# raphaelsulzer/PixelsPointsPolygons

Hardware: NVIDIA B200
Metric: pillar_encode_tiles_per_sec (higher is better)
Workload: dtype f16 operands, f32 accumulate, f32 in/out

## Files before the change

### pixelspointspolygons_b200/csrc/voxelize.cu

```cuda
#include <type_traits>

#include "p3p_internal.cuh"

namespace p3p {

#ifdef P3P_TIMELINE
__device__ unsigned long long g_timeline[8192][16];
__device__ __forceinline__ void tl_stamp(int cta, int slot) {
    if (threadIdx.x == 0 && cta < 8192) {
        unsigned long long t;
        asm volatile("mov.u64 %0, %%globaltimer;" : "=l"(t));
        g_timeline[cta][slot] = t;
    }
}
#define TL(cta, slot) tl_stamp(cta, slot)
extern "C" int p3p_debug_timeline(unsigned long long* host, int ctas) {
    return (int)cudaMemcpyFromSymbol(host, g_timeline, sizeof(unsigned long long) * 16 * (size_t)ctas);
}
#else
#define TL(cta, slot)
#endif

namespace {

constexpr int kThreads = kVoxThreads;
constexpr int kWarps = kThreads / 32;
constexpr int kIters = kMaxChunkPoints / kThreads;

struct ChunkLoc {
    int b;
    int c;
    int nchunks;
    int gstart;
    long long p0;
    long long lo, hi;
    unsigned sat;
};

__device__ __forceinline__ unsigned atoms_add_u16(uint32_t addr, int pred) {
    unsigned r;
    const unsigned sh = (addr & 2u) * 8u;
    asm volatile(
        "{\n .reg .pred p;\n setp.ne.b32 p, %3, 0;\n mov.b32 %0, 0;\n @p atom.shared.add.u32 %0, [%1], %2;\n}"
        : "=r"(r)
        : "r"(addr & ~3u), "r"(1u << sh), "r"(pred)
        : "memory");
    return (r >> sh) & 0xFFFFu;
}

__device__ __forceinline__ unsigned ld_acquire(const unsigned* p) {
    unsigned v;
    asm volatile("ld.acquire.gpu.global.u32 %0, [%1];" : "=r"(v) : "l"(p) : "memory");
    return v;
}
__device__ __forceinline__ void st_release(unsigned* p, unsigned v) {
    asm volatile("st.release.gpu.global.u32 [%0], %1;" ::"l"(p), "r"(v) : "memory");
}

__device__ void locate_chunk(int g, const int64_t* __restrict__ offsets, int B, int S, int phase, ChunkLoc* out) {
    const int lane = threadIdx.x & 31;
    if (B <= 32) {
        long long o0 = 0, o1 = 0;
        if (lane < B) { o0 = offsets[lane]; o1 = offsets[lane + 1]; }
        const long long a0 = o0 - ((o0 - phase) & 3ll);
        const long long n = o1 > o0 ? o1 - a0 : 0;
        const int nc = (int)((n + S - 1) / S);
        int incl = nc;
#pragma unroll
        for (int o = 1; o < 32; o <<= 1) {
            const int v = __shfl_up_sync(0xffffffffu, incl, o);
            if (lane >= o) incl += v;
        }
        const int total = __shfl_sync(0xffffffffu, incl, 31);
        if (g >= total) {
            if (lane == 0) out->b = -1;
            return;
        }
        int lo = 0, hi = __reduce_max_sync(0xffffffffu, nc) - 1;
        while (lo < hi) {
            const int mid = (lo + hi + 1) >> 1;
            if (__reduce_add_sync(0xffffffffu, nc < mid ? nc : mid) <= g) lo = mid; else hi = mid - 1;
        }
        const int c = lo;
        const int r = g - __reduce_add_sync(0xffffffffu, nc < c ? nc : c);
        const bool has = nc > c;
        const unsigned bal = __ballot_sync(0xffffffffu, has);
        if (has && __popc(bal & ((1u << lane) - 1u)) == r) {
            out->b = lane;
            out->c = c;
            out->nchunks = nc;
            out->gstart = incl - nc;
            out->p0 = a0 + (long long)c * S;
            out->lo = o0;
            out->hi = o1;
        }
        return;
    }
    int base = 0;
    bool found = false;
    for (int t0 = 0; t0 < B && !found; t0 += 32) {
        const int t = t0 + lane;
        long long o0 = 0, o1 = 0;
        if (t < B) { o0 = offsets[t]; o1 = offsets[t + 1]; }
        const long long a0 = o0 - ((o0 - phase) & 3ll);
        const long long n = o1 > o0 ? o1 - a0 : 0;
        const int nc = (int)((n + S - 1) / S);
        int incl = nc;
#pragma unroll
        for (int o = 1; o < 32; o <<= 1) {
            const int v = __shfl_up_sync(0xffffffffu, incl, o);
            if (lane >= o) incl += v;
        }
        const int excl = base + incl - nc;
        const bool mine = (t < B) && (g >= excl) && (g < excl + nc);
        const unsigned bal = __ballot_sync(0xffffffffu, mine);
        if (bal) {
            found = true;
            if (mine) {
                out->b = t;
                out->c = g - excl;
                out->nchunks = nc;
                out->gstart = excl;
                out->p0 = a0 + (long long)(g - excl) * S;
                out->lo = o0;
                out->hi = o1;
            }
        }
        base += __shfl_sync(0xffffffffu, incl, 31);
    }
    if (!found && lane == 0) out->b = -1;
}

__device__ __forceinline__ int block_exclusive_scan(int v, int* warp_tot, int* total) {
    const int lane = threadIdx.x & 31, w = threadIdx.x >> 5;
    int incl = v;
#pragma unroll
    for (int o = 1; o < 32; o <<= 1) {
        const int t = __shfl_up_sync(0xffffffffu, incl, o);
        if (lane >= o) incl += t;
    }
    __syncthreads();
    if (lane == 31) warp_tot[w] = incl;
    __syncthreads();
    int off = 0, tot = 0;
#pragma unroll
    for (int i = 0; i < kWarps; ++i) {
        const int t = warp_tot[i];
        if (i < w) off += t;
        tot += t;
    }
    *total = tot;
    return off + incl - v;
}

__device__ void write_empty_tile(const GridDev& g, const WsPtrs& ws, int b) {
    const int HW = g.ny * g.nx;
    for (int i = threadIdx.x; i < HW; i += kThreads) {
        ws.owner[(size_t)b * HW + i] = -1;
        ws.cell_desc[(size_t)b * HW + i] = -1;
    }
    if (threadIdx.x == 0) ws.num_pil[b] = 0;
}

__device__ void plan_tile(const GridDev& g, const WsPtrs& ws, int b, int Keff, int* scratch, int* warp_tot) {
    const int K = g.num_keys, HW = g.ny * g.nx, M = g.M, tid = threadIdx.x;
    int* n_s = scratch;
    int* cell_s = n_s + K;
    int* rkey_s = cell_s + K;
    int* rn_s = rkey_s + K;
    int* owner_s = rn_s + K;
    const int* totals = ws.totals + (size_t)b * K;
    const float4* slots = ws.slots + (size_t)b * K * M;
    const uint8_t* edge = ws.edge + (size_t)b * K;
    for (int k0 = 0; k0 < Keff; k0 += kThreads * 8) {
        int t[8];
        uint8_t e[8];
#pragma unroll
        for (int u = 0; u < 8; ++u) {
            const int k = k0 + u * kThreads + tid;
            t[u] = 0; e[u] = 0;
            if (k < Keff) { t[u] = __ldcg(totals + k); e[u] = __ldcg(edge + k); }
        }
#pragma unroll
        for (int u = 0; u < 8; ++u) {
            const int k = k0 + u * kThreads + tid;
            if (k >= Keff) continue;
            int cell = -1;
            const int n = t[u] < M ? t[u] : M;
            if (n > 0) {
                int cx, cy, cz;
                if (e[u]) {
                    float4 best = __ldcg(slots + (size_t)k * M);
                    for (int i = 1; i < n; ++i) {
                        const float4 p = __ldcg(slots + (size_t)k * M + i);
                        if (__float_as_int(p.w) < __float_as_int(best.w)) best = p;
                    }
                    point_cell(g, best.x, best.y, best.z, cx, cy, cz);
                } else {
                    cz = k / g.stride2;
                    const int rem = k - cz * g.stride2;
                    cy = rem / g.stride1;
                    cx = rem - cy * g.stride1;
                }
                if (cy < g.nv[1] && cx < g.nv[0]) cell = cx | (cy << 10) | (cz << 20);
            }
            n_s[k] = n;
            cell_s[k] = cell;
        }
    }
    for (int i = tid; i < HW; i += kThreads) owner_s[i] = -1;
    __syncthreads();
    const int per = (Keff + kThreads - 1) / kThreads;
    const int k0 = tid * per, k1 = (k0 + per < Keff) ? k0 + per : Keff;
    int cnt = 0;
    for (int k = k0; k < k1; ++k) cnt += (n_s[k] > 0);
    int total_runs;
    int ord = block_exclusive_scan(cnt, warp_tot, &total_runs);
    int cnt2 = 0;
    for (int k = k0; k < k1; ++k) {
        if (n_s[k] > 0) {
            const int r = ord++;
            if (r >= g.Vmax) cell_s[k] = -1;
        }
        cnt2 += (cell_s[k] >= 0);
    }
    int total_pil;
    int ord2 = block_exclusive_scan(cnt2, warp_tot, &total_pil);
    for (int k = k0; k < k1; ++k) {
        const int st = cell_s[k];
        if (st < 0) continue;
        const int r = ord2++;
        const size_t pi = (size_t)b * g.Vmax + r;
        const int n = n_s[k];
        ws.pil_key[pi] = k;
        ws.pil_n[pi] = n;
        ws.pil_coord[pi] = st;
        rkey_s[r] = k;
        rn_s[r] = n;
        const int cx = st & 1023, cy = (st >> 10) & 1023;
        atomicMax(&owner_s[cy * g.nx + cx], r);
    }
    if (tid == 0) ws.num_pil[b] = total_pil;
    __syncthreads();
    for (int i = tid; i < HW; i += kThreads) {
        const int o = owner_s[i];
        ws.owner[(size_t)b * HW + i] = o;
        ws.cell_desc[(size_t)b * HW + i] = (o >= 0) ? (rkey_s[o] | (rn_s[o] << 16)) : -1;
    }
}

constexpr int kKeyBits = 13;
constexpr unsigned kKeyMask = (1u << kKeyBits) - 1u;
static_assert(kMaxKeys <= (1 << kKeyBits), "key field too narrow");
static_assert(kMaxChunkPoints * 8 < 65536, "8 chunk rows must add up inside 16-bit lanes");
constexpr int kGroups = kIters / 4;
#ifndef P3P_CROSS_BATCH
#define P3P_CROSS_BATCH 256
#endif
constexpr int kCrossBatch = P3P_CROSS_BATCH;
constexpr int kCells = kGroups * kWarps;
static_assert(kMaxChunkPoints / kCells <= 255, "points of a cell must fit the 8-bit fields of the boundary word");
constexpr unsigned kCrossFlag = 0x8000u;

template <bool kFast>
__global__ void __launch_bounds__(kThreads, kVoxCtasPerSm)
voxelize_kernel(const float* __restrict__ pts, int stride_arg, const int64_t* __restrict__ offsets, int B, GridDev g, int S, WsPtrs ws, int32_t* __restrict__ point_hash, int need_plan, int pdl_from) {
    extern __shared__ __align__(16) unsigned char smem_raw[];
    const int K = g.num_keys;
    const int Kp = ws.key_stride;
    uint16_t* ctot_s = reinterpret_cast<uint16_t*>(smem_raw);
    uint16_t* base_s = ctot_s + Kp;
    uint16_t* need_s = base_s + Kp;
    unsigned* bnd_s = reinterpret_cast<unsigned*>(need_s + Kp);
    uint16_t* cell_s = reinterpret_cast<uint16_t*>(bnd_s + kCrossBatch);
    __shared__ ChunkLoc loc;
    __shared__ int s_ticket, s_last, s_runs[2], s_ncross;
    __shared__ int warp_tot[kWarps];

    const int tid = threadIdx.x, lane = tid & 31;
    const int stride = kFast ? 3 : stride_arg;
    TL(blockIdx.x, 0);
    if (tid == 0) { s_ticket = (int)atomicAdd(ws.sync, 1u); s_ncross = 0; }
    {
        uint4* h4 = reinterpret_cast<uint4*>(ctot_s);
        for (int i = tid; i < Kp / 8; i += kThreads) h4[i] = make_uint4(0, 0, 0, 0);
    }
    __syncthreads();
    const int ticket = s_ticket;
    if (ticket >= pdl_from) asm volatile("griddepcontrol.launch_dependents;" ::: "memory");
    unsigned* flags = ws.sync + 1;
    unsigned* tile_done = flags + ws.max_chunks;
    unsigned* tile_sat = tile_done + B;
    if (tid < 32) {
        locate_chunk(ticket, offsets, B, S, kFast ? (int)((reinterpret_cast<uintptr_t>(pts) >> 2) & 3u) : 0, &loc);
        __syncwarp();
        if (lane == 0 && loc.b >= 0) loc.sat = __ldcg(tile_sat + loc.b);
    }
    if (ticket < B && offsets[ticket + 1] <= offsets[ticket]) write_empty_tile(g, ws, ticket);
    __syncthreads();
    if (loc.b < 0) return;
    TL(blockIdx.x, 1);

    uint8_t* edge = ws.edge + (size_t)loc.b * K;
    const int M = g.M;
    const unsigned sat_word = loc.sat;
    const bool saturated = sat_word != 0u && (int)(0x7fffffffu - sat_word) < loc.c;

    int pk[kIters];
    int hi_key = 0;
    const long long lo = loc.lo, hi = loc.hi;
    const uint32_t ctot_sa = smem_u32(ctot_s);
    const bool interior = kFast && S == kMaxChunkPoints && loc.p0 >= lo && loc.p0 + S <= hi;
    auto load_group = [&](int gi, float (&x)[4], float (&y)[4], float (&z)[4]) {
        const long long p = loc.p0 + 4ll * (kThreads * gi + tid);
        if (kFast && p >= lo && p + 4 <= hi) {
            const float4* q = reinterpret_cast<const float4*>(pts + p * 3);
            const float4 a = __ldg(q), b = __ldg(q + 1), c = __ldg(q + 2);
            x[0] = a.x; y[0] = a.y; z[0] = a.z; x[1] = a.w; y[1] = b.x; z[1] = b.y;
            x[2] = b.z; y[2] = b.w; z[2] = c.x; x[3] = c.y; y[3] = c.z; z[3] = c.w;
        } else {
#pragma unroll
            for (int e = 0; e < 4; ++e) {
                x[e] = y[e] = z[e] = __int_as_float(0x7fc00000);
                if (p + e >= lo && p + e < hi) {
                    const float* q = pts + (p + e) * stride;
                    x[e] = __ldg(q); y[e] = __ldg(q + 1); z[e] = __ldg(q + 2);
                }
            }
        }
    };
    {
        unsigned edge_bits = 0;
        int kmax = -1;
        auto hash_group = [&](int gi, const float (&x)[4], const float (&y)[4], const float (&z)[4]) {
#pragma unroll
            for (int e = 0; e < 4; ++e) {
                bool on_edge;
                int k = point_key<!kFast>(g, x[e], y[e], z[e], on_edge);
                if (!kFast && point_hash) {
                    const long long p = loc.p0 + 4ll * (kThreads * gi + tid) + e;
                    if (p >= lo && p < hi) point_hash[p] = k;
                }
                edge_bits |= on_edge ? (1u << (4 * gi + e)) : 0u;
                kmax = k > kmax ? k : kmax;
                if (saturated && k < g.num_cells) k = -1;
                pk[4 * gi + e] = k;
            }
        };
        if (interior) {
            const float4* q = reinterpret_cast<const float4*>(pts + (loc.p0 + 4ll * tid) * 3);
            float4 v[kGroups][3];
#pragma unroll
            for (int gi = 0; gi < kGroups; ++gi) {
#pragma unroll
                for (int u = 0; u < 3; ++u) v[gi][u] = __ldg(q + (size_t)gi * (kThreads * 3) + u);
            }
#pragma unroll
            for (int gi = 0; gi < kGroups; ++gi) {
                const float4 a = v[gi][0], b = v[gi][1], c = v[gi][2];
                const float x[4] = {a.x, a.w, b.z, c.y}, y[4] = {a.y, b.x, b.w, c.z}, z[4] = {a.z, b.y, c.x, c.w};
                hash_group(gi, x, y, z);
            }
        } else {
#pragma unroll
            for (int gi = 0; gi < kGroups; ++gi) {
                if (4 * kThreads * gi < S) {
                    float x[4], y[4], z[4];
                    load_group(gi, x, y, z);
                    hash_group(gi, x, y, z);
                } else {
#pragma unroll
                    for (int e = 0; e < 4; ++e) pk[4 * gi + e] = -1;
                }
            }
        }
        hi_key |= ((kmax >= g.num_cells) ? 1 : 0) | (edge_bits ? 3 : 0);
        if (edge_bits) {
#pragma unroll
            for (int j = 0; j < kIters; ++j)
                if (((edge_bits >> j) & 1u) && pk[j] >= 0) edge[pk[j]] = 1;
        }
        TL(blockIdx.x, 2);
#pragma unroll
        for (int j = 0; j < kIters; ++j) {
            const int k = pk[j];
            const int act = k >= 0 ? 1 : 0;
            const unsigned old = atoms_add_u16(ctot_sa + 2u * (unsigned)(act ? k : 0), act);
            if (act) pk[j] = k | (int)(old << kKeyBits);
        }
    }
    hi_key = (__syncthreads_or(hi_key & 1) ? 1 : 0) | (__syncthreads_or(hi_key & 2) ? 2 : 0);
    TL(blockIdx.x, 3);
    if (tid < 2) s_runs[tid] = 0;
    const int Kreg = (g.num_cells + 7) / 8 * 8 < Kp ? (g.num_cells + 7) / 8 * 8 : Kp;
    {
        uint4* dst = reinterpret_cast<uint4*>(ws.chunk_hist + (size_t)(loc.gstart + loc.c) * Kp);
        for (int k8 = tid; k8 < Kp / 8; k8 += kThreads) dst[k8] = reinterpret_cast<const uint4*>(ctot_s)[k8];
        __syncthreads();
        if (tid == 0) {
            __threadfence();
            st_release(flags + loc.gstart + loc.c, 1u | ((unsigned)hi_key << 1));
        }
        TL(blockIdx.x, 4);
        int hi_before = 0;
        for (int cc = tid; cc < loc.c; cc += kThreads) {
            unsigned f;
            while ((f = ld_acquire(flags + loc.gstart + cc)) == 0u) {
            }
            hi_before |= (int)(f >> 1);
        }
        hi_key |= (__syncthreads_or(hi_before & 1) ? 1 : 0) | (__syncthreads_or(hi_before & 2) ? 2 : 0);
    }
    TL(blockIdx.x, 5);
    const bool last_chunk = (loc.c == loc.nchunks - 1);
    const int Kuse = (hi_key & 1) ? Kp : Kreg;
    int open_keys = 0;
    int all_full = 1;
    for (int k8 = tid; k8 < Kp / 8; k8 += kThreads) {
        unsigned acc[8] = {0, 0, 0, 0, 0, 0, 0, 0};
        if (k8 * 8 < Kuse && !(saturated && k8 * 8 + 8 <= g.num_cells)) {
            const uint4* src = reinterpret_cast<const uint4*>(ws.chunk_hist + (size_t)loc.gstart * Kp) + k8;
            const size_t row = (size_t)Kp / 8;
            const uint4* rp = src;
            auto add_rows = [&](const uint4 (&v)[8]) {
                uint4 sum = v[0];
#pragma unroll
                for (int u = 1; u < 8; ++u) { sum.x += v[u].x; sum.y += v[u].y; sum.z += v[u].z; sum.w += v[u].w; }
                acc[0] += sum.x & 0xFFFFu; acc[1] += sum.x >> 16; acc[2] += sum.y & 0xFFFFu; acc[3] += sum.y >> 16;
                acc[4] += sum.z & 0xFFFFu; acc[5] += sum.z >> 16; acc[6] += sum.w & 0xFFFFu; acc[7] += sum.w >> 16;
            };
            int c0 = 0;
            for (; c0 + 8 <= loc.c; c0 += 8, rp += 8 * row) {
                uint4 v[8];
#pragma unroll
                for (int u = 0; u < 8; ++u) v[u] = __ldcg(rp + u * row);
                add_rows(v);
            }
            if (c0 < loc.c) {
                uint4 v[8];
#pragma unroll
                for (int u = 0; u < 8; ++u) v[u] = (c0 + u < loc.c) ? __ldcg(rp + u * row) : make_uint4(0, 0, 0, 0);
                add_rows(v);
            }
        }
#pragma unroll
        for (int u = 0; u < 8; ++u) {
            const int k = k8 * 8 + u;
            const unsigned own = ctot_s[k];
            unsigned pre = acc[u];
            if (saturated && k < g.num_cells) pre = (unsigned)M;
            unsigned st = pre < (unsigned)M ? pre : (unsigned)M;
            if (own > 0 && pre < (unsigned)M) {
                open_keys = 1;
                if (pre + own > (unsigned)M) {
                    const unsigned id = (unsigned)atomicAdd(&s_ncross, 1);
                    need_s[id] = (uint16_t)((unsigned)M - pre);
                    st = kCrossFlag | id;
                }
            }
            base_s[k] = (uint16_t)st;
            if (k < g.num_cells && pre + own < (unsigned)M) all_full = 0;
            if (last_chunk) {
                const unsigned tot = pre + own;
                if (k < K) ws.totals[(size_t)loc.b * K + k] = (int)tot;
                ctot_s[k] = (uint16_t)(tot < (unsigned)M ? tot : (unsigned)M);
            }
        }
    }
    open_keys = __syncthreads_or(open_keys);
    all_full = __syncthreads_and(all_full);
    if (all_full && !saturated && !last_chunk && tid == 0) atomicMax(tile_sat + loc.b, 0x7fffffffu - (unsigned)loc.c);
    TL(blockIdx.x, 6);
    if (last_chunk) {
        int direct = 0, hi_ok = 0;
        if (!need_plan && !(hi_key & 2)) {
            int r = 0, h = 0;
            for (int k = tid; k < Kuse && k < K; k += kThreads) {
                const int nz = ctot_s[k] > 0 ? 1 : 0;
                if (k < g.num_cells) r += nz; else h += nz;
            }
            r = __reduce_add_sync(0xffffffffu, r);
            h = __reduce_add_sync(0xffffffffu, h);
            if (lane == 0) { atomicAdd(&s_runs[0], r); atomicAdd(&s_runs[1], h); }
            __syncthreads();
            const int R = s_runs[0], H = s_runs[1];
            hi_ok = (R + H <= g.Vmax) ? 1 : 0;
            direct = (R <= g.Vmax) && (H == 0 || hi_ok || R == g.Vmax);
        }
        if (direct) {
            const int HW = g.ny * g.nx;
            const int top = hi_ok ? g.ext[2] : g.ext[2] - 1;
            for (int cell = tid; cell < HW; cell += kThreads) {
                const int cy = cell / g.nx, cx = cell - cy * g.nx;
                int d = -1;
                if (cx < g.nv[0] && cy < g.nv[1]) {
                    for (int cz = top; cz >= 0; --cz) {
                        const int k = cx + cy * g.stride1 + cz * g.stride2;
                        const int n = (k < Kuse && k < K) ? (int)ctot_s[k] : 0;
                        if (n > 0) { d = k | (n << 16); break; }
                    }
                }
                ws.cell_desc[(size_t)loc.b * HW + cell] = d;
            }
        }
        if (tid == 0) ws.tile_hi[loc.b] = (hi_key & 1) | (direct << 1);
    }
    float4* tile_slots = ws.slots + (size_t)loc.b * K * M;
    unsigned xmask = 0;
    const int w = tid >> 5;
    if (open_keys) {
#pragma unroll
        for (int j = 0; j < kIters; ++j) {
            if (pk[j] >= 0) {
                const unsigned key = (unsigned)pk[j] & kKeyMask;
                const unsigned st = base_s[key];
                if (st & kCrossFlag) xmask |= 1u << j;
                else if (st < (unsigned)M) pk[j] = (int)(key | ((st + ((unsigned)pk[j] >> kKeyBits)) << kKeyBits));
                else pk[j] = -1;
            }
        }
    } else {
#pragma unroll
        for (int j = 0; j < kIters; ++j) pk[j] = -1;
    }
    TL(blockIdx.x, 7);
    const int ncross = s_ncross;
    for (int c0 = 0; c0 < ncross; c0 += kCrossBatch) {
        const int nb = ncross - c0 < kCrossBatch ? ncross - c0 : kCrossBatch;
        {
            uint4* c4 = reinterpret_cast<uint4*>(cell_s);
            for (int i = tid; i < kCells * kCrossBatch / 8; i += kThreads) c4[i] = make_uint4(0, 0, 0, 0);
        }
        __syncthreads();
        const uint32_t cell_sa = smem_u32(cell_s);
        unsigned bmask = 0;
        if (xmask) {
#pragma unroll
            for (int j = 0; j < kIters; ++j) {
                if ((xmask >> j) & 1u) {
                    const unsigned key = (unsigned)pk[j] & kKeyMask;
                    const int id = (int)(base_s[key] & (kCrossFlag - 1u)) - c0;
                    if (id >= 0 && id < nb) {
                        bmask |= 1u << j;
                        const unsigned cell = (unsigned)((j >> 2) * kWarps + w);
                        const unsigned local = atoms_add_u16(cell_sa + 2u * (cell * kCrossBatch + (unsigned)id), 1);
                        pk[j] = (int)(key | (local << kKeyBits));
                    }
                }
            }
        }
        __syncthreads();
        for (int id = tid; id < nb; id += kThreads) {
            const unsigned need = need_s[c0 + id];
            unsigned P = 0, bnd = 0;
            bool found = false;
#pragma unroll 8
            for (int c = 0; c < kCells; ++c) {
                const unsigned v = cell_s[c * kCrossBatch + id];
                cell_s[c * kCrossBatch + id] = (uint16_t)P;
                if (!found && P + v >= need) { found = true; bnd = (unsigned)c | ((need - P) << 8) | (v << 16); }
                P += v;
            }
            bnd_s[id] = bnd;
        }
        __syncthreads();
        if (__any_sync(0xffffffffu, bmask != 0)) {
#pragma unroll
            for (int gi = 0; gi < kGroups; ++gi) {
                const unsigned cell = (unsigned)(gi * kWarps + w);
                unsigned flag = 0;
                int keyv[4];
#pragma unroll
                for (int e = 0; e < 4; ++e) {
                    const int j = 4 * gi + e;
                    keyv[e] = -1;
                    if ((bmask >> j) & 1u) {
                        const unsigned key = (unsigned)pk[j] & kKeyMask, local = (unsigned)pk[j] >> kKeyBits;
                        const int id = (int)(base_s[key] & (kCrossFlag - 1u)) - c0;
                        const unsigned bnd = bnd_s[id], bc = bnd & 0xFFu, rem = (bnd >> 8) & 0xFFu, cnt = bnd >> 16;
                        const unsigned pre = (unsigned)M - need_s[c0 + id];
                        const unsigned P = cell_s[cell * kCrossBatch + (unsigned)id];
                        if (cell < bc || (cell == bc && rem == cnt)) pk[j] = (int)(key | ((pre + P + local) << kKeyBits));
                        else if (cell > bc) pk[j] = -1;
                        else { flag |= 1u << e; keyv[e] = (int)key; }
                    }
                }
                unsigned pending = __ballot_sync(0xffffffffu, flag != 0);
                while (pending) {
                    const int leader = __ffs(pending) - 1;
                    const int mine = (flag & 1u) ? keyv[0] : ((flag & 2u) ? keyv[1] : ((flag & 4u) ? keyv[2] : keyv[3]));
                    const int kk = __shfl_sync(0xffffffffu, mine, leader);
                    unsigned b[4], m = 0;
#pragma unroll
                    for (int e = 0; e < 4; ++e) {
                        const bool hit = ((flag >> e) & 1u) && keyv[e] == kk;
                        m |= hit ? (1u << e) : 0u;
                        b[e] = __ballot_sync(0xffffffffu, hit);
                    }
                    if (m) {
                        const int id = (int)(base_s[kk] & (kCrossFlag - 1u)) - c0;
                        const unsigned rem = (bnd_s[id] >> 8) & 0xFFu;
                        const unsigned pre = (unsigned)M - need_s[c0 + id];
                        const unsigned P = cell_s[cell * kCrossBatch + (unsigned)id];
                        const unsigned lt = (1u << lane) - 1u;
                        unsigned below = (unsigned)(__popc(b[0] & lt) + __popc(b[1] & lt) + __popc(b[2] & lt) + __popc(b[3] & lt));
#pragma unroll
                        for (int e = 0; e < 4; ++e) {
                            if ((m >> e) & 1u) {
                                pk[4 * gi + e] = below < rem ? (int)((unsigned)kk | ((pre + P + below) << kKeyBits)) : -1;
                                ++below;
                            }
                        }
                        flag &= ~m;
                    }
                    pending = __ballot_sync(0xffffffffu, flag != 0);
                }
            }
        }
        xmask &= ~bmask;
        __syncthreads();
    }
    TL(blockIdx.x, 8);
    {
        unsigned live = 0;
#pragma unroll
        for (int j = 0; j < kIters; ++j) live |= (pk[j] >= 0) ? (1u << (j >> 2)) : 0u;
        if (interior) {
            const float4* q = reinterpret_cast<const float4*>(pts + (loc.p0 + 4ll * tid) * 3);
#pragma unroll
            for (int h = 0; h < kGroups; h += 2) {
                float4 v[2][3];
#pragma unroll
                for (int g2 = 0; g2 < 2; ++g2) {
                    if (h + g2 < kGroups && ((live >> (h + g2)) & 1u)) {
#pragma unroll
                        for (int u = 0; u < 3; ++u) v[g2][u] = __ldg(q + (size_t)(h + g2) * (kThreads * 3) + u);
                    }
                }
#pragma unroll
                for (int g2 = 0; g2 < 2; ++g2) {
                    const int gi = (h + g2 < kGroups) ? h + g2 : kGroups - 1;
                    if (h + g2 < kGroups && ((live >> gi) & 1u)) {
                        const float4 a = v[g2][0], b = v[g2][1], c = v[g2][2];
                        const float x[4] = {a.x, a.w, b.z, c.y}, y[4] = {a.y, b.x, b.w, c.z}, z[4] = {a.z, b.y, c.x, c.w};
#pragma unroll
                        for (int e = 0; e < 4; ++e) {
                            const int j = 4 * gi + e;
                            if (pk[j] >= 0) {
                                const int ci = 4 * (kThreads * gi + tid) + e;
                                tile_slots[(size_t)((unsigned)pk[j] & kKeyMask) * M + ((unsigned)pk[j] >> kKeyBits)] =
                                    make_float4(x[e], y[e], z[e], __int_as_float((int)(loc.p0 + ci - lo)));
                            }
                        }
                    }
                }
            }
        } else {
#pragma unroll
            for (int gi = 0; gi < kGroups; ++gi) {
                if ((live >> gi) & 1u) {
                    float x[4], y[4], z[4];
                    load_group(gi, x, y, z);
#pragma unroll
                    for (int e = 0; e < 4; ++e) {
                        const int j = 4 * gi + e;
                        if (pk[j] >= 0) {
                            const int ci = 4 * (kThreads * gi + tid) + e;
                            tile_slots[(size_t)((unsigned)pk[j] & kKeyMask) * M + ((unsigned)pk[j] >> kKeyBits)] =
                                make_float4(x[e], y[e], z[e], __int_as_float((int)(loc.p0 + ci - lo)));
                        }
                    }
                }
            }
        }
    }
    __syncthreads();
    TL(blockIdx.x, 9);
    if (tid == 0) {
        __threadfence();
        s_last = (atomicAdd(tile_done + loc.b, 1u) == (unsigned)(loc.nchunks - 1)) ? 1 : 0;
        __threadfence();
    }
    __syncthreads();
    if (!s_last) return;
    TL(blockIdx.x, 10);
    const int tile_hi = __ldcg(ws.tile_hi + loc.b);
    if (tile_hi & 2) return;
    plan_tile(g, ws, loc.b, (tile_hi & 1) ? K : (g.num_cells < K ? g.num_cells : K), reinterpret_cast<int*>(smem_raw), warp_tot);
    __syncthreads();
    TL(blockIdx.x, 11);
}

__global__ void __launch_bounds__(128)
export_kernel(GridDev g, int B, WsPtrs ws, p3p_voxel_outputs out) {
    __shared__ int idx_s[1024];
    const int b = blockIdx.y;
    const int HW = g.ny * g.nx;
    const int np = ws.num_pil[b];
    if (blockIdx.x == 0) {
        if (out.num_pillars && threadIdx.x == 0) out.num_pillars[b] = np;
        if (out.cell_owner)
            for (int i = threadIdx.x; i < HW; i += blockDim.x) out.cell_owner[(size_t)b * HW + i] = ws.owner[(size_t)b * HW + i];
    }
    for (int r = blockIdx.x; r < np; r += gridDim.x) {
        const size_t pi = (size_t)b * g.Vmax + r;
        const int key = ws.pil_key[pi], n = ws.pil_n[pi], pc = ws.pil_coord[pi];
        if (threadIdx.x == 0) {
            if (out.pillar_coords) {
                int* c = out.pillar_coords + pi * 4;
                c[0] = b; c[1] = pc >> 20; c[2] = (pc >> 10) & 1023; c[3] = pc & 1023;
            }
            if (out.pillar_num_points) out.pillar_num_points[pi] = n;
        }
        const float4* slot = ws.slots + ((size_t)b * g.num_keys + key) * g.M;
        __syncthreads();
        for (int s = threadIdx.x; s < n; s += blockDim.x) idx_s[s] = __float_as_int(slot[s].w);
        __syncthreads();
        for (int s = threadIdx.x; s < g.M; s += blockDim.x) {
            int pos = s;
            float4 p = make_float4(0.f, 0.f, 0.f, __int_as_float(-1));
            if (s < n) {
                p = slot[s];
                const int me = idx_s[s];
                pos = 0;
                for (int i = 0; i < n; ++i) pos += (idx_s[i] < me) ? 1 : 0;
            }
            if (out.pillar_point_idx) out.pillar_point_idx[pi * g.M + pos] = __float_as_int(p.w);
            if (out.pillar_points) {
                float* d = out.pillar_points + (pi * g.M + pos) * 3;
                d[0] = p.x; d[1] = p.y; d[2] = p.z;
            }
        }
    }
}

}

size_t voxelize_smem_bytes(const GridDev& g) {
    const size_t kp = ((size_t)g.num_keys + 7) / 8 * 8;
    const size_t rank = 3 * kp * sizeof(uint16_t) + kCrossBatch * sizeof(unsigned) + (size_t)kCells * kCrossBatch * sizeof(uint16_t);
    const size_t plan = (size_t)(4 * g.num_keys + g.ny * g.nx) * sizeof(int);
    return ((rank > plan ? rank : plan) + 15) / 16 * 16;
}

int launch_voxelize(const float* pts, int stride, const int64_t* offsets, int B, int64_t total, const GridDev& g,
                    const WsLayout& l, const WsPtrs& ws, int32_t* point_hash, int need_plan, cudaStream_t st) {
    (void)total;
    const size_t smem = voxelize_smem_bytes(g);
    if (smem > kVoxelizeMaxSmem) return fail(P3P_ERR_UNSUPPORTED, "voxel grid needs %zu bytes of shared memory per CTA (limit %zu)", smem, kVoxelizeMaxSmem);
    P3P_CUDA_CHECK(cudaFuncSetAttribute(voxelize_kernel<true>, cudaFuncAttributeMaxDynamicSharedMemorySize, (int)kVoxelizeMaxSmem));
    P3P_CUDA_CHECK(cudaFuncSetAttribute(voxelize_kernel<false>, cudaFuncAttributeMaxDynamicSharedMemorySize, (int)kVoxelizeMaxSmem));
    P3P_CUDA_CHECK(cudaMemsetAsync(ws.sync, 0, l.sync_bytes, st));
    const int pdl_from = l.max_chunks - device_sm_count();
    if (stride == 3 && point_hash == nullptr && !(g.flags & kFlagDropOverflow))
        voxelize_kernel<true><<<l.max_chunks, kThreads, smem, st>>>(pts, stride, offsets, B, g, l.chunk_points, ws, point_hash, need_plan, pdl_from);
    else
        voxelize_kernel<false><<<l.max_chunks, kThreads, smem, st>>>(pts, stride, offsets, B, g, l.chunk_points, ws, point_hash, need_plan, pdl_from);
    P3P_CUDA_CHECK(cudaGetLastError());
    return P3P_OK;
}

int launch_export(const GridDev& g, int B, const WsPtrs& ws, const p3p_voxel_outputs* out, cudaStream_t st) {
    dim3 grid((unsigned)(g.Vmax < 256 ? (g.Vmax > 0 ? g.Vmax : 1) : 256), (unsigned)B);
    export_kernel<<<grid, 128, 0, st>>>(g, B, ws, *out);
    P3P_CUDA_CHECK(cudaGetLastError());
    return P3P_OK;
}

}
```

Measured before the change: 303,200.

## Rank points with per-warp key counters and deterministic order, dropping cross-key fixup

Each warp now owns a contiguous span of the chunk and counts keys in a private 16-bit histogram in shared memory. Ranks within the warp come from match_any and popc over a staged group of 128 points. A per-key exclusive scan across warps turns these into slot positions that already follow point order. This removes the shared-atomic ranking, the batched cross-boundary fixup that decided which points fill a nearly full pillar, and the O(n^2) sort by index in the export kernel. In exchange it needs kWarps times more shared histogram memory, which can lower occupancy, and adds a reduction and scan across warps over all keys.

Measured after the change: 275,600, median of 6. 9.1% lower.

```diff
diff --git a/pixelspointspolygons_b200/csrc/voxelize.cu b/pixelspointspolygons_b200/csrc/voxelize.cu
--- a/pixelspointspolygons_b200/csrc/voxelize.cu
+++ b/pixelspointspolygons_b200/csrc/voxelize.cu
@@ -14,11 +14,14 @@
     }
 }
 #define TL(cta, slot) tl_stamp(cta, slot)
+#define TLV(cta, slot, v) \
+    do { if (threadIdx.x == 0 && (cta) < 8192) g_timeline[cta][slot] = (unsigned long long)(v); } while (0)
 extern "C" int p3p_debug_timeline(unsigned long long* host, int ctas) {
     return (int)cudaMemcpyFromSymbol(host, g_timeline, sizeof(unsigned long long) * 16 * (size_t)ctas);
 }
 #else
 #define TL(cta, slot)
+#define TLV(cta, slot, v)
 #endif
 
 namespace {
@@ -36,17 +39,6 @@
     long long lo, hi;
     unsigned sat;
 };
-
-__device__ __forceinline__ unsigned atoms_add_u16(uint32_t addr, int pred) {
-    unsigned r;
-    const unsigned sh = (addr & 2u) * 8u;
-    asm volatile(
-        "{\n .reg .pred p;\n setp.ne.b32 p, %3, 0;\n mov.b32 %0, 0;\n @p atom.shared.add.u32 %0, [%1], %2;\n}"
-        : "=r"(r)
-        : "r"(addr & ~3u), "r"(1u << sh), "r"(pred)
-        : "memory");
-    return (r >> sh) & 0xFFFFu;
-}
 
 __device__ __forceinline__ unsigned ld_acquire(const unsigned* p) {
     unsigned v;
@@ -253,14 +245,9 @@
 constexpr unsigned kKeyMask = (1u << kKeyBits) - 1u;
 static_assert(kMaxKeys <= (1 << kKeyBits), "key field too narrow");
 static_assert(kMaxChunkPoints * 8 < 65536, "8 chunk rows must add up inside 16-bit lanes");
+static_assert(1024 + kMaxChunkPoints < 65536, "min(pre, M) + a chunk's points must fit a 16-bit counter (M <= 1024, capi.cu)");
 constexpr int kGroups = kIters / 4;
-#ifndef P3P_CROSS_BATCH
-#define P3P_CROSS_BATCH 256
-#endif
-constexpr int kCrossBatch = P3P_CROSS_BATCH;
-constexpr int kCells = kGroups * kWarps;
-static_assert(kMaxChunkPoints / kCells <= 255, "points of a cell must fit the 8-bit fields of the boundary word");
-constexpr unsigned kCrossFlag = 0x8000u;
+constexpr int kGroupPoints = 128;
 
 template <bool kFast>
 __global__ void __launch_bounds__(kThreads, kVoxCtasPerSm)
@@ -268,22 +255,20 @@
     extern __shared__ __align__(16) unsigned char smem_raw[];
     const int K = g.num_keys;
     const int Kp = ws.key_stride;
-    uint16_t* ctot_s = reinterpret_cast<uint16_t*>(smem_raw);
-    uint16_t* base_s = ctot_s + Kp;
-    uint16_t* need_s = base_s + Kp;
-    unsigned* bnd_s = reinterpret_cast<unsigned*>(need_s + Kp);
-    uint16_t* cell_s = reinterpret_cast<uint16_t*>(bnd_s + kCrossBatch);
+    int* stage_s = reinterpret_cast<int*>(smem_raw);
+    uint16_t* cnt_s = reinterpret_cast<uint16_t*>(stage_s + kWarps * kGroupPoints);
+    uint16_t* ctot_s = cnt_s + (size_t)kWarps * Kp;
     __shared__ ChunkLoc loc;
-    __shared__ int s_ticket, s_last, s_runs[2], s_ncross;
+    __shared__ int s_ticket, s_last, s_runs[2];
     __shared__ int warp_tot[kWarps];
 
-    const int tid = threadIdx.x, lane = tid & 31;
+    const int tid = threadIdx.x, lane = tid & 31, w = tid >> 5;
     const int stride = kFast ? 3 : stride_arg;
     TL(blockIdx.x, 0);
-    if (tid == 0) { s_ticket = (int)atomicAdd(ws.sync, 1u); s_ncross = 0; }
+    if (tid == 0) s_ticket = (int)atomicAdd(ws.sync, 1u);
     {
-        uint4* h4 = reinterpret_cast<uint4*>(ctot_s);
-        for (int i = tid; i < Kp / 8; i += kThreads) h4[i] = make_uint4(0, 0, 0, 0);
+        uint4* c4 = reinterpret_cast<uint4*>(cnt_s);
+        for (int i = tid; i < kWarps * Kp / 8; i += kThreads) c4[i] = make_uint4(0, 0, 0, 0);
     }
     __syncthreads();
     const int ticket = s_ticket;
@@ -300,6 +285,8 @@
     __syncthreads();
     if (loc.b < 0) return;
     TL(blockIdx.x, 1);
+    TLV(blockIdx.x, 12, loc.c + 1);
+    TLV(blockIdx.x, 13, loc.b + 1);
 
     uint8_t* edge = ws.edge + (size_t)loc.b * K;
     const int M = g.M;
@@ -309,10 +296,11 @@
     int pk[kIters];
     int hi_key = 0;
     const long long lo = loc.lo, hi = loc.hi;
-    const uint32_t ctot_sa = smem_u32(ctot_s);
+    const int wspan = S / kWarps;
+    const long long pw = loc.p0 + (long long)wspan * w + 4 * lane;
     const bool interior = kFast && S == kMaxChunkPoints && loc.p0 >= lo && loc.p0 + S <= hi;
     auto load_group = [&](int gi, float (&x)[4], float (&y)[4], float (&z)[4]) {
-        const long long p = loc.p0 + 4ll * (kThreads * gi + tid);
+        const long long p = pw + kGroupPoints * gi;
         if (kFast && p >= lo && p + 4 <= hi) {
             const float4* q = reinterpret_cast<const float4*>(pts + p * 3);
             const float4 a = __ldg(q), b = __ldg(q + 1), c = __ldg(q + 2);
@@ -338,7 +326,7 @@
                 bool on_edge;
                 int k = point_key<!kFast>(g, x[e], y[e], z[e], on_edge);
                 if (!kFast && point_hash) {
-                    const long long p = loc.p0 + 4ll * (kThreads * gi + tid) + e;
+                    const long long p = pw + kGroupPoints * gi + e;
                     if (p >= lo && p < hi) point_hash[p] = k;
                 }
                 edge_bits |= on_edge ? (1u << (4 * gi + e)) : 0u;
@@ -348,12 +336,12 @@
             }
         };
         if (interior) {
-            const float4* q = reinterpret_cast<const float4*>(pts + (loc.p0 + 4ll * tid) * 3);
+            const float4* q = reinterpret_cast<const float4*>(pts + pw * 3);
             float4 v[kGroups][3];
 #pragma unroll
             for (int gi = 0; gi < kGroups; ++gi) {
 #pragma unroll
-                for (int u = 0; u < 3; ++u) v[gi][u] = __ldg(q + (size_t)gi * (kThreads * 3) + u);
+                for (int u = 0; u < 3; ++u) v[gi][u] = __ldg(q + gi * (kGroupPoints * 3 / 4) + u);
             }
 #pragma unroll
             for (int gi = 0; gi < kGroups; ++gi) {
@@ -364,7 +352,7 @@
         } else {
 #pragma unroll
             for (int gi = 0; gi < kGroups; ++gi) {
-                if (4 * kThreads * gi < S) {
+                if (kGroupPoints * gi < wspan) {
                     float x[4], y[4], z[4];
                     load_group(gi, x, y, z);
                     hash_group(gi, x, y, z);
@@ -380,13 +368,36 @@
             for (int j = 0; j < kIters; ++j)
                 if (((edge_bits >> j) & 1u) && pk[j] >= 0) edge[pk[j]] = 1;
         }
-        TL(blockIdx.x, 2);
-#pragma unroll
-        for (int j = 0; j < kIters; ++j) {
-            const int k = pk[j];
-            const int act = k >= 0 ? 1 : 0;
-            const unsigned old = atoms_add_u16(ctot_sa + 2u * (unsigned)(act ? k : 0), act);
-            if (act) pk[j] = k | (int)(old << kKeyBits);
+    }
+    TL(blockIdx.x, 2);
+    {
+        int* stage = stage_s + w * kGroupPoints;
+        uint16_t* cnt = cnt_s + (size_t)w * Kp;
+        const unsigned lt = (1u << lane) - 1u;
+#pragma unroll
+        for (int gi = 0; gi < kGroups; ++gi) {
+            if (kGroupPoints * gi >= wspan) break;
+            reinterpret_cast<int4*>(stage)[lane] = make_int4(pk[4 * gi], pk[4 * gi + 1], pk[4 * gi + 2], pk[4 * gi + 3]);
+            __syncwarp();
+            int key[4];
+            unsigned m[4];
+#pragma unroll
+            for (int r = 0; r < 4; ++r) key[r] = stage[32 * r + lane];
+#pragma unroll
+            for (int r = 0; r < 4; ++r) m[r] = __match_any_sync(0xffffffffu, key[r]);
+#pragma unroll
+            for (int r = 0; r < 4; ++r) {
+                const int leader = __ffs(m[r]) - 1;
+                const bool lead = lane == leader && key[r] >= 0;
+                unsigned c = lead ? (unsigned)cnt[key[r]] : 0u;
+                c = __shfl_sync(0xffffffffu, c, leader);
+                if (lead) cnt[key[r]] = (uint16_t)(c + (unsigned)__popc(m[r]));
+                if (key[r] >= 0) stage[32 * r + lane] = key[r] | (int)((c + (unsigned)__popc(m[r] & lt)) << kKeyBits);
+                __syncwarp();
+            }
+            const int4 v = reinterpret_cast<const int4*>(stage)[lane];
+            pk[4 * gi] = v.x; pk[4 * gi + 1] = v.y; pk[4 * gi + 2] = v.z; pk[4 * gi + 3] = v.w;
+            __syncwarp();
         }
     }
     hi_key = (__syncthreads_or(hi_key & 1) ? 1 : 0) | (__syncthreads_or(hi_key & 2) ? 2 : 0);
@@ -395,7 +406,17 @@
     const int Kreg = (g.num_cells + 7) / 8 * 8 < Kp ? (g.num_cells + 7) / 8 * 8 : Kp;
     {
         uint4* dst = reinterpret_cast<uint4*>(ws.chunk_hist + (size_t)(loc.gstart + loc.c) * Kp);
-        for (int k8 = tid; k8 < Kp / 8; k8 += kThreads) dst[k8] = reinterpret_cast<const uint4*>(ctot_s)[k8];
+        const uint4* c4 = reinterpret_cast<const uint4*>(cnt_s);
+        for (int k8 = tid; k8 < Kp / 8; k8 += kThreads) {
+            uint4 s = c4[k8];
+#pragma unroll
+            for (int v = 1; v < kWarps; ++v) {
+                const uint4 t = c4[v * (Kp / 8) + k8];
+                s.x += t.x; s.y += t.y; s.z += t.z; s.w += t.w;
+            }
+            reinterpret_cast<uint4*>(ctot_s)[k8] = s;
+            dst[k8] = s;
+        }
         __syncthreads();
         if (tid == 0) {
             __threadfence();
@@ -443,27 +464,32 @@
                 add_rows(v);
             }
         }
+        unsigned base[4] = {0, 0, 0, 0};
+        int in_chunk = 0;
 #pragma unroll
         for (int u = 0; u < 8; ++u) {
             const int k = k8 * 8 + u;
             const unsigned own = ctot_s[k];
             unsigned pre = acc[u];
             if (saturated && k < g.num_cells) pre = (unsigned)M;
-            unsigned st = pre < (unsigned)M ? pre : (unsigned)M;
-            if (own > 0 && pre < (unsigned)M) {
-                open_keys = 1;
-                if (pre + own > (unsigned)M) {
-                    const unsigned id = (unsigned)atomicAdd(&s_ncross, 1);
-                    need_s[id] = (uint16_t)((unsigned)M - pre);
-                    st = kCrossFlag | id;
-                }
-            }
-            base_s[k] = (uint16_t)st;
+            base[u >> 1] |= (pre < (unsigned)M ? pre : (unsigned)M) << (16 * (u & 1));
+            in_chunk |= own > 0 ? 1 : 0;
+            if (own > 0 && pre < (unsigned)M) open_keys = 1;
             if (k < g.num_cells && pre + own < (unsigned)M) all_full = 0;
             if (last_chunk) {
                 const unsigned tot = pre + own;
                 if (k < K) ws.totals[(size_t)loc.b * K + k] = (int)tot;
                 ctot_s[k] = (uint16_t)(tot < (unsigned)M ? tot : (unsigned)M);
+            }
+        }
+        if (in_chunk) {
+            uint4 run = make_uint4(base[0], base[1], base[2], base[3]);
+            uint4* c4 = reinterpret_cast<uint4*>(cnt_s) + k8;
+#pragma unroll
+            for (int v = 0; v < kWarps; ++v) {
+                const uint4 t = c4[v * (Kp / 8)];
+                c4[v * (Kp / 8)] = run;
+                run.x += t.x; run.y += t.y; run.z += t.z; run.w += t.w;
             }
         }
     }
@@ -506,17 +532,15 @@
         if (tid == 0) ws.tile_hi[loc.b] = (hi_key & 1) | (direct << 1);
     }
     float4* tile_slots = ws.slots + (size_t)loc.b * K * M;
-    unsigned xmask = 0;
-    const int w = tid >> 5;
+    const int pl = (int)(pw - lo);
     if (open_keys) {
+        const uint16_t* off = cnt_s + (size_t)w * Kp;
 #pragma unroll
         for (int j = 0; j < kIters; ++j) {
             if (pk[j] >= 0) {
                 const unsigned key = (unsigned)pk[j] & kKeyMask;
-                const unsigned st = base_s[key];
-                if (st & kCrossFlag) xmask |= 1u << j;
-                else if (st < (unsigned)M) pk[j] = (int)(key | ((st + ((unsigned)pk[j] >> kKeyBits)) << kKeyBits));
-                else pk[j] = -1;
+                const unsigned r = off[key] + ((unsigned)pk[j] >> kKeyBits);
+                pk[j] = r < (unsigned)M ? (int)(key | (r << kKeyBits)) : -1;
             }
         }
     } else {
@@ -524,109 +548,12 @@
         for (int j = 0; j < kIters; ++j) pk[j] = -1;
     }
     TL(blockIdx.x, 7);
-    const int ncross = s_ncross;
-    for (int c0 = 0; c0 < ncross; c0 += kCrossBatch) {
-        const int nb = ncross - c0 < kCrossBatch ? ncross - c0 : kCrossBatch;
-        {
-            uint4* c4 = reinterpret_cast<uint4*>(cell_s);
-            for (int i = tid; i < kCells * kCrossBatch / 8; i += kThreads) c4[i] = make_uint4(0, 0, 0, 0);
-        }
-        __syncthreads();
-        const uint32_t cell_sa = smem_u32(cell_s);
-        unsigned bmask = 0;
-        if (xmask) {
-#pragma unroll
-            for (int j = 0; j < kIters; ++j) {
-                if ((xmask >> j) & 1u) {
-                    const unsigned key = (unsigned)pk[j] & kKeyMask;
-                    const int id = (int)(base_s[key] & (kCrossFlag - 1u)) - c0;
-                    if (id >= 0 && id < nb) {
-                        bmask |= 1u << j;
-                        const unsigned cell = (unsigned)((j >> 2) * kWarps + w);
-                        const unsigned local = atoms_add_u16(cell_sa + 2u * (cell * kCrossBatch + (unsigned)id), 1);
-                        pk[j] = (int)(key | (local << kKeyBits));
-                    }
-                }
-            }
-        }
-        __syncthreads();
-        for (int id = tid; id < nb; id += kThreads) {
-            const unsigned need = need_s[c0 + id];
-            unsigned P = 0, bnd = 0;
-            bool found = false;
-#pragma unroll 8
-            for (int c = 0; c < kCells; ++c) {
-                const unsigned v = cell_s[c * kCrossBatch + id];
-                cell_s[c * kCrossBatch + id] = (uint16_t)P;
-                if (!found && P + v >= need) { found = true; bnd = (unsigned)c | ((need - P) << 8) | (v << 16); }
-                P += v;
-            }
-            bnd_s[id] = bnd;
-        }
-        __syncthreads();
-        if (__any_sync(0xffffffffu, bmask != 0)) {
-#pragma unroll
-            for (int gi = 0; gi < kGroups; ++gi) {
-                const unsigned cell = (unsigned)(gi * kWarps + w);
-                unsigned flag = 0;
-                int keyv[4];
-#pragma unroll
-                for (int e = 0; e < 4; ++e) {
-                    const int j = 4 * gi + e;
-                    keyv[e] = -1;
-                    if ((bmask >> j) & 1u) {
-                        const unsigned key = (unsigned)pk[j] & kKeyMask, local = (unsigned)pk[j] >> kKeyBits;
-                        const int id = (int)(base_s[key] & (kCrossFlag - 1u)) - c0;
-                        const unsigned bnd = bnd_s[id], bc = bnd & 0xFFu, rem = (bnd >> 8) & 0xFFu, cnt = bnd >> 16;
-                        const unsigned pre = (unsigned)M - need_s[c0 + id];
-                        const unsigned P = cell_s[cell * kCrossBatch + (unsigned)id];
-                        if (cell < bc || (cell == bc && rem == cnt)) pk[j] = (int)(key | ((pre + P + local) << kKeyBits));
-                        else if (cell > bc) pk[j] = -1;
-                        else { flag |= 1u << e; keyv[e] = (int)key; }
-                    }
-                }
-                unsigned pending = __ballot_sync(0xffffffffu, flag != 0);
-                while (pending) {
-                    const int leader = __ffs(pending) - 1;
-                    const int mine = (flag & 1u) ? keyv[0] : ((flag & 2u) ? keyv[1] : ((flag & 4u) ? keyv[2] : keyv[3]));
-                    const int kk = __shfl_sync(0xffffffffu, mine, leader);
-                    unsigned b[4], m = 0;
-#pragma unroll
-                    for (int e = 0; e < 4; ++e) {
-                        const bool hit = ((flag >> e) & 1u) && keyv[e] == kk;
-                        m |= hit ? (1u << e) : 0u;
-                        b[e] = __ballot_sync(0xffffffffu, hit);
-                    }
-                    if (m) {
-                        const int id = (int)(base_s[kk] & (kCrossFlag - 1u)) - c0;
-                        const unsigned rem = (bnd_s[id] >> 8) & 0xFFu;
-                        const unsigned pre = (unsigned)M - need_s[c0 + id];
-                        const unsigned P = cell_s[cell * kCrossBatch + (unsigned)id];
-                        const unsigned lt = (1u << lane) - 1u;
-                        unsigned below = (unsigned)(__popc(b[0] & lt) + __popc(b[1] & lt) + __popc(b[2] & lt) + __popc(b[3] & lt));
-#pragma unroll
-                        for (int e = 0; e < 4; ++e) {
-                            if ((m >> e) & 1u) {
-                                pk[4 * gi + e] = below < rem ? (int)((unsigned)kk | ((pre + P + below) << kKeyBits)) : -1;
-                                ++below;
-                            }
-                        }
-                        flag &= ~m;
-                    }
-                    pending = __ballot_sync(0xffffffffu, flag != 0);
-                }
-            }
-        }
-        xmask &= ~bmask;
-        __syncthreads();
-    }
-    TL(blockIdx.x, 8);
     {
         unsigned live = 0;
 #pragma unroll
         for (int j = 0; j < kIters; ++j) live |= (pk[j] >= 0) ? (1u << (j >> 2)) : 0u;
         if (interior) {
-            const float4* q = reinterpret_cast<const float4*>(pts + (loc.p0 + 4ll * tid) * 3);
+            const float4* q = reinterpret_cast<const float4*>(pts + pw * 3);
 #pragma unroll
             for (int h = 0; h < kGroups; h += 2) {
                 float4 v[2][3];
@@ -634,7 +561,7 @@
                 for (int g2 = 0; g2 < 2; ++g2) {
                     if (h + g2 < kGroups && ((live >> (h + g2)) & 1u)) {
 #pragma unroll
-                        for (int u = 0; u < 3; ++u) v[g2][u] = __ldg(q + (size_t)(h + g2) * (kThreads * 3) + u);
+                        for (int u = 0; u < 3; ++u) v[g2][u] = __ldg(q + (h + g2) * (kGroupPoints * 3 / 4) + u);
                     }
                 }
 #pragma unroll
@@ -647,9 +574,8 @@
                         for (int e = 0; e < 4; ++e) {
                             const int j = 4 * gi + e;
                             if (pk[j] >= 0) {
-                                const int ci = 4 * (kThreads * gi + tid) + e;
                                 tile_slots[(size_t)((unsigned)pk[j] & kKeyMask) * M + ((unsigned)pk[j] >> kKeyBits)] =
-                                    make_float4(x[e], y[e], z[e], __int_as_float((int)(loc.p0 + ci - lo)));
+                                    make_float4(x[e], y[e], z[e], __int_as_float(pl + kGroupPoints * gi + e));
                             }
                         }
                     }
@@ -665,9 +591,8 @@
                     for (int e = 0; e < 4; ++e) {
                         const int j = 4 * gi + e;
                         if (pk[j] >= 0) {
-                            const int ci = 4 * (kThreads * gi + tid) + e;
                             tile_slots[(size_t)((unsigned)pk[j] & kKeyMask) * M + ((unsigned)pk[j] >> kKeyBits)] =
-                                make_float4(x[e], y[e], z[e], __int_as_float((int)(loc.p0 + ci - lo)));
+                                make_float4(x[e], y[e], z[e], __int_as_float(pl + kGroupPoints * gi + e));
                         }
                     }
                 }
@@ -675,7 +600,7 @@
         }
     }
     __syncthreads();
-    TL(blockIdx.x, 9);
+    TL(blockIdx.x, 8);
     if (tid == 0) {
         __threadfence();
         s_last = (atomicAdd(tile_done + loc.b, 1u) == (unsigned)(loc.nchunks - 1)) ? 1 : 0;
@@ -683,17 +608,16 @@
     }
     __syncthreads();
     if (!s_last) return;
-    TL(blockIdx.x, 10);
+    TL(blockIdx.x, 9);
     const int tile_hi = __ldcg(ws.tile_hi + loc.b);
     if (tile_hi & 2) return;
     plan_tile(g, ws, loc.b, (tile_hi & 1) ? K : (g.num_cells < K ? g.num_cells : K), reinterpret_cast<int*>(smem_raw), warp_tot);
     __syncthreads();
-    TL(blockIdx.x, 11);
+    TL(blockIdx.x, 10);
 }
 
 __global__ void __launch_bounds__(128)
 export_kernel(GridDev g, int B, WsPtrs ws, p3p_voxel_outputs out) {
-    __shared__ int idx_s[1024];
     const int b = blockIdx.y;
     const int HW = g.ny * g.nx;
     const int np = ws.num_pil[b];
@@ -713,21 +637,11 @@
             if (out.pillar_num_points) out.pillar_num_points[pi] = n;
         }
         const float4* slot = ws.slots + ((size_t)b * g.num_keys + key) * g.M;
-        __syncthreads();
-        for (int s = threadIdx.x; s < n; s += blockDim.x) idx_s[s] = __float_as_int(slot[s].w);
-        __syncthreads();
         for (int s = threadIdx.x; s < g.M; s += blockDim.x) {
-            int pos = s;
-            float4 p = make_float4(0.f, 0.f, 0.f, __int_as_float(-1));
-            if (s < n) {
-                p = slot[s];
-                const int me = idx_s[s];
-                pos = 0;
-                for (int i = 0; i < n; ++i) pos += (idx_s[i] < me) ? 1 : 0;
-            }
-            if (out.pillar_point_idx) out.pillar_point_idx[pi * g.M + pos] = __float_as_int(p.w);
+            const float4 p = s < n ? slot[s] : make_float4(0.f, 0.f, 0.f, __int_as_float(-1));
+            if (out.pillar_point_idx) out.pillar_point_idx[pi * g.M + s] = __float_as_int(p.w);
             if (out.pillar_points) {
-                float* d = out.pillar_points + (pi * g.M + pos) * 3;
+                float* d = out.pillar_points + (pi * g.M + s) * 3;
                 d[0] = p.x; d[1] = p.y; d[2] = p.z;
             }
         }
@@ -738,7 +652,7 @@
 
 size_t voxelize_smem_bytes(const GridDev& g) {
     const size_t kp = ((size_t)g.num_keys + 7) / 8 * 8;
-    const size_t rank = 3 * kp * sizeof(uint16_t) + kCrossBatch * sizeof(unsigned) + (size_t)kCells * kCrossBatch * sizeof(uint16_t);
+    const size_t rank = (size_t)kWarps * kGroupPoints * sizeof(int) + (size_t)(kWarps + 1) * kp * sizeof(uint16_t);
     const size_t plan = (size_t)(4 * g.num_keys + g.ny * g.nx) * sizeof(int);
     return ((rank > plan ? rank : plan) + 15) / 16 * 16;
 }
```
